# tomwhite/disq

Hardware: AMD Instinct MI355X
Metric: decompressed BAM GB/s + reads/sec (whole node) at 1/2/4/8 MI355X (higher is better)
Workload: dtype u8

## Files before the change

disq_amd/csrc/dq_inflate3.hip:

```cpp
#include "dq_inflate_core.h"
#include "dq_internal.h"

#include <mutex>
#include <vector>

namespace dq {
namespace {

using namespace dqi;

#define DQ_HD __device__ __host__ __attribute__((always_inline)) inline

#ifndef DQ_BLK_WG
#define DQ_BLK_WG 512
#endif
constexpr int WG = DQ_BLK_WG;
static_assert(WG % 128 == 0 && WG >= 512 && WG <= 1024, "whole waves on every SIMD");
constexpr int NWV = WG / 64;
constexpr int NDEC = WG;
constexpr uint32_t OV_DEFAULT = 96;
#ifndef DQ_TAIL_OV
#define DQ_TAIL_OV OV_DEFAULT
#endif
constexpr int OUTCAP = 65536 + 24;
#ifndef DQ_CSTEP
#define DQ_CSTEP 0
#endif
#ifndef DQ_RES_NB
#define DQ_RES_NB (WG == 512 ? 4 : 2)
#endif
#ifndef DQ_RES_G
#define DQ_RES_G 1
#endif
#ifndef DQ_RES_QUAD
#define DQ_RES_QUAD 1
#endif
constexpr int RES_NXT = DQ_RES_NB * DQ_RES_G * WG;
constexpr int NCARRY = (65536 + RES_NXT - 1) / RES_NXT + 1;


constexpr int LR = 10, DR = 8;
constexpr int LSB = 15 - LR, DSB = 15 - DR;
constexpr int LSLOTS = 16, DSLOTS = 4;
constexpr int MAXGRP = 64;
constexpr int T_LSUB = 1 << LR;
constexpr int T_DROOT = T_LSUB + LSLOTS * (1 << LSB);
constexpr int T_DSUB = T_DROOT + (1 << DR);
constexpr int T_END = T_DSUB + DSLOTS * (1 << DSB);
constexpr int HB_WORDS = 160;
constexpr uint16_t E_SLOW = 0x0080;
constexpr uint32_t LL_EOB = 0xF810, LL_BAD = 0xF910;
DQ_HD uint16_t ent_ll(uint32_t sym, uint32_t len) {
  if (sym < 256) return (uint16_t)(sym << 8 | len);
  if (sym == 256) return (uint16_t)(LL_EOB | len);
  if (sym > 285) return (uint16_t)(LL_BAD | len);
  const uint32_t k = sym - 257;
  const uint32_t x = (k < 8 || k == 28) ? 0u : (k - 4) >> 2;
  const uint32_t base = k < 8 ? k + 3 : k == 28 ? 258u : ((4u + (k & 3u)) << ((k - 4) >> 2)) + 3u;
  return (uint16_t)((base - 3) << 8 | x << 5 | 16u | len);
}
DQ_HD uint16_t ent_d(uint32_t d, uint32_t len) {
  if (d >= 30) return (uint16_t)(0x4000u | len);
  const uint32_t x = d < 4 ? 0u : (d - 2) >> 1;
  const uint32_t m = d < 2 ? d : 2u + (d & 1u), sh = d < 2 ? 0u : (d >> 1) - 1u;
  return (uint16_t)(m << 12 | sh << 8 | x << 4 | len);
}

enum : int32_t { F_EXIT = 0, F_EOB = 1, F_ERR = 2, F_END = 3 };

constexpr int TOUT = 4096;
constexpr int TAIL_MAX_BITS = 32768;
constexpr int TW = 4;
#ifndef DQ_ROOT_REG
#define DQ_ROOT_REG 1
#endif
#ifndef DQ_TAIL_HDR1
#define DQ_TAIL_HDR1 1
#endif
constexpr int T_NCK = 4;
#ifndef DQ_TAIL_SEG
#define DQ_TAIL_SEG 96
#endif
constexpr int TAIL_SEG_MIN = DQ_TAIL_SEG;
constexpr int TIM_W = 32;
struct TailDesc {
  int32_t pos;
  int32_t produced;
  uint32_t crc_raw;
  int32_t flag;
};

struct alignas(16) LdsI {
  static constexpr int kLSUB = T_LSUB, kDROOT = T_DROOT, kDSUB = T_DSUB;
  [[maybe_unused]] static constexpr int kTEND = T_END;
  static constexpr bool kPair = true;
  alignas(8) uint32_t bm[2048];
  union {
    struct {
      uint16_t T[T_END];
      HuffCanon hl, hd;
      uint16_t lend[16], dend[16];
      uint16_t lent[288];
      uint16_t dent[32];
      union {
        uint16_t pair[1 << LR];
        struct {
          uint8_t lens[320];
          uint8_t clen[20];
          uint16_t clt[128];
          union {
            struct {
              int32_t cntw[NWV];
              int32_t cnts[NWV];
              uint32_t ginfo[MAXGRP + 32];
              uint32_t cntp[8][8];
              uint16_t pref[320];
            };
            struct {
              uint8_t exitm[NWV][16];
              int32_t ent[NWV + 1];
              int32_t wt[NWV];
              int32_t lv[NWV];
              int32_t endp;
            };
          };
        } h;
      } x;
    } d;
    struct {
      uint16_t last_start[1024];
      uint16_t nxt[RES_NXT];
      int32_t carry_ms[NCARRY];
      uint32_t carry_desc[NCARRY];
    } r;
    uint32_t crc4[4][256];
  } u;
  int32_t misc[32];
  union {
    struct {
      int32_t wsum[16];
      int32_t small[8 * 7];
    };
    uint32_t scratch[16 + 8 * 7];
  };
  alignas(16) uint8_t out[OUTCAP];
};
static_assert(sizeof(((LdsI*)nullptr)->scratch) >= 64 * 4, "one emit dummy word per lane");
static_assert(offsetof(LdsI, out) < 65536 - 4096, "the tables' offsets fit the DS offset field");
static_assert(2 * sizeof(LdsI) <= 160 * 1024, "two workgroups per CU");
static_assert(HB_WORDS * 4 <= T_END * 2, "header staging fits the decode table");

__device__ inline uint32_t* emit_dummy(LdsI& L) { return L.scratch; }

__constant__ uint32_t c_crc4[4][256];
__constant__ uint32_t c_x2n[32];
__constant__ uint32_t c_x8n[TOUT + 1];
constexpr int CRC_SL = 4 * (((65536 / 4 + WG - 1) / WG) | 1);
static_assert(CRC_SL * WG >= 65536, "the slices cover the largest block");
__constant__ uint32_t c_slice_shift[WG];
__constant__ uint8_t c_clorder3[19] = {16, 17, 18, 0, 8, 7, 9, 6, 10, 5, 11, 4, 12, 3, 13, 2, 14, 1, 15};

enum { M_ERR = 0, M_SLOW = 1 , M_A = 4, M_LAST, M_MORE, M_MORE1,
       M_LQ0 = 15, M_LQN, M_DQ0, M_DQN, M_NEXT,
       M_LASTF, M_RCNT = 28 ,
       M_DIRTY = 30  };

template <class LT>
__device__ __attribute__((always_inline)) inline void set_err(LT& L, int32_t code) { atomicCAS(&L.misc[M_ERR], 0, code); }


#define DQ_AI __device__ __attribute__((always_inline)) inline

DQ_AI int tid_fresh() {
  int t = (int)threadIdx.x;
  asm volatile("" : "+v"(t));
  return t;
}

typedef uint32_t u32x4 __attribute__((ext_vector_type(4)));
DQ_AI void st_nt(uint4* d, uint4 v) {
  u32x4 x = {v.x, v.y, v.z, v.w};
  __builtin_nontemporal_store(x, reinterpret_cast<u32x4*>(d));
}

struct GSrc {
  const uint32_t* __restrict__ p;
#ifdef DQ_CHECKED
  uint32_t lim;
  uint32_t tag;
#endif
  DQ_AI uint32_t operator[](uint32_t i) const {
#ifdef DQ_CHECKED
    DQ_CHKV(i < lim, CHK_K2_BITS, tag | min(i - lim + 1, 4095u));
#endif
    return *reinterpret_cast<const uint32_t*>(reinterpret_cast<const uint8_t*>(p) + (i << 2));
  }
};

#ifndef DQ_BR64
#define DQ_BR64 0
#endif
#if DQ_BR64
struct BitR {
  uint64_t bb;
  uint32_t bc;
  uint32_t wp;
  uint32_t nw;
};
template <class S>
DQ_AI void br_init(BitR& r, const S& W, uint32_t bitpos) {
  const uint32_t wi = bitpos >> 5;
  const uint64_t lo = W[wi], hi = W[wi + 1];
  const uint32_t sh = bitpos & 31;
  r.bb = ((hi << 32) | lo) >> sh;
  r.bc = 64 - sh;
  r.wp = wi + 2;
  r.nw = W[r.wp];
}
template <class S>
DQ_AI void br_refill(BitR& r, const S& W) {
  const bool need = r.bc <= 32;
  r.bb |= (uint64_t)(need ? r.nw : 0u) << r.bc;
  r.bc += need ? 32u : 0u;
  r.wp += need ? 1u : 0u;
  r.nw = W[r.wp];
}
DQ_AI uint32_t br_pos(const BitR& r) { return r.wp * 32 - r.bc; }
DQ_AI uint32_t br_peek(const BitR& r) { return (uint32_t)r.bb; }
template <class S>
DQ_AI void br_take(BitR& r, const S&, uint32_t n) {
  r.bb >>= n;
  r.bc -= n;
}
#else
struct BitR {
  uint32_t p;
  uint32_t w0, w1;
  uint32_t nw;
};
template <class S>
DQ_AI void br_init(BitR& r, const S& W, uint32_t bitpos) {
  const uint32_t wi = bitpos >> 5;
  r.w0 = W[wi];
  r.w1 = W[wi + 1];
  r.nw = W[wi + 2];
  r.p = bitpos;
}
template <class S>
DQ_AI void br_refill(BitR&, const S&) {}
DQ_AI uint32_t br_pos(const BitR& r) { return r.p; }
DQ_AI uint32_t br_peek(const BitR& r) { return __builtin_amdgcn_alignbit(r.w1, r.w0, r.p); }
template <class S>
DQ_AI void br_take(BitR& r, const S& W, uint32_t n) {
  const uint32_t q = r.p + n;
  const bool c = (q ^ r.p) >= 32u;
  r.w0 = c ? r.w1 : r.w0;
  r.w1 = c ? r.nw : r.w1;
  r.p = q;
  r.nw = W[(q >> 5) + 2];
}
#endif
DQ_AI uint32_t peek_bits(const uint32_t* __restrict__ W, uint32_t pos, uint32_t n) {
  const uint32_t wi = pos >> 5;
  const uint64_t v = ((uint64_t)W[wi + 1] << 32) | W[wi];
  return (uint32_t)(v >> (pos & 31)) & ((1u << n) - 1);
}

template <class LT>
DQ_AI uint32_t load_desc(const LT& L, int a) {
  const uint32_t* w = reinterpret_cast<const uint32_t*>(L.out + (a & ~3));
  return __builtin_amdgcn_alignbyte(w[1], w[0], (uint32_t)a & 3u) & 0xffffffu;
}

DQ_AI uint32_t zx16(uint16_t v) {
#ifndef DQ_NO_ZX16
  uint32_t x = v;
  asm("" : "+v"(x));
  return x;
#else
  return v;
#endif
}

template <bool SLOW, class LT>
DQ_AI uint32_t ll_second(const LT& L, uint32_t e, uint32_t bb) {
  const uint32_t sb = (e >> 4) & 7;
  DQ_CHK(LT::kLSUB + (e >> 7) + ((bb >> LR) & ((1u << sb) - 1)) < (uint32_t)LT::kDROOT, CHK_K2_TABLE);
  if (!SLOW) return L.u.d.T[LT::kLSUB + (e >> 7) + ((bb >> LR) & ((1u << sb) - 1))];
  if (sb) return L.u.d.T[LT::kLSUB + (e >> 7) + ((bb >> LR) & ((1u << sb) - 1))];
  if (!(e & E_SLOW)) return 0u;
  int l = 0;
  const int k = canon_decode(bb, L.u.d.hl, LR + 1, &l);
  return k < 0 ? 0u : L.u.d.lent[k];
}
template <bool SLOW, class LT>
DQ_AI uint32_t d_second(const LT& L, uint32_t e, uint32_t bb) {
  const uint32_t sb = (e >> 4) & 7;
  DQ_CHK(LT::kDSUB + (e >> 7) + ((bb >> DR) & ((1u << sb) - 1)) < (uint32_t)LT::kTEND, CHK_K2_TABLE);
  if (!SLOW) return L.u.d.T[LT::kDSUB + (e >> 7) + ((bb >> DR) & ((1u << sb) - 1))];
  if (sb) return L.u.d.T[LT::kDSUB + (e >> 7) + ((bb >> DR) & ((1u << sb) - 1))];
  if (!(e & E_SLOW)) return 0u;
  int l = 0;
  const int k = canon_decode(bb, L.u.d.hd, DR + 1, &l);
  return k < 0 ? 0u : L.u.d.dent[k];
}


template <bool SLOW, class S, class LT>
DQ_AI bool dsym(BitR& r, const S& W, const LT& L, uint32_t p, uint32_t lim,
                uint32_t& len, uint32_t& dist, uint32_t& lit2, bool& is_m, uint32_t& e) {
  br_refill(r, W);
  uint32_t bb = br_peek(r);
  const uint32_t ri = bb & ((1u << LR) - 1);
  e = L.u.d.T[ri];
  uint32_t pe = 0;
  if constexpr (LT::kPair) pe = zx16(L.u.d.x.pair[ri]);
  if ((e & 15) == 0) e = ll_second<SLOW>(L, e, bb);
  const uint32_t nb = e & 15;
  const uint32_t lx = __builtin_amdgcn_ubfe(e, 5, 3);
  is_m = (e & 16) != 0;
  len = (e >> 8) + (is_m ? 3u : 0u) + __builtin_amdgcn_ubfe(bb, nb, lx);
  const bool two = pe != 0 && p + nb < lim;
  lit2 = two ? pe >> 8 : 0xffffffffu;
  br_take(r, W, nb + lx + (two ? (pe & 15) : 0u));
  br_refill(r, W);
  bb = br_peek(r);
  uint32_t e2 = zx16(L.u.d.T[LT::kDROOT + (bb & ((1u << DR) - 1))]);
  if (is_m && (e2 & 15) == 0) e2 = d_second<SLOW>(L, e2, bb);
  const uint32_t nb2 = e2 & 15, dx = __builtin_amdgcn_ubfe(e2, 4, 4);
  dist = (__builtin_amdgcn_ubfe(e2, 12, 2) << __builtin_amdgcn_ubfe(e2, 8, 4)) + 1u +
         __builtin_amdgcn_ubfe(bb, nb2, dx);
  br_take(r, W, is_m ? nb2 + dx : 0u);
  return (SLOW && nb == 0) || (e & 0xFEF0u) == 0xF810u ||
         (is_m && ((SLOW && nb2 == 0) || (e2 & 0x4000u)));
}
DQ_AI uint32_t stop_end(uint32_t e, uint32_t p) {
  return (e & 15) != 0 && (e & 0xFFF0u) == LL_EOB ? p + (e & 15) : 0xffffffffu;
}

enum : int32_t { F_DEAD = 4 };

constexpr int NCK_DEFAULT = 8;
constexpr uint32_t CKI_DEFAULT = 48;

template <bool SLOW, class S, class LT>
DQ_AI int run_seg(const S& W, const LT& L, uint32_t start, uint32_t sB,
                  uint32_t sE, uint32_t endbits, int32_t* Bp, int32_t* Ep, int32_t* cntp,
                  uint32_t* ck, int ckstride, uint32_t CKI, int NCK) {
  BitR r;
  br_init(r, W, start);
  uint32_t p = br_pos(r);
  uint32_t len = 0, dist = 0, lit2, e = 0;
  bool m;
  const uint32_t sBe = min(sB, endbits);
  while (p < sBe) {
    if (dsym<SLOW>(r, W, L, p, sBe, len, dist, lit2, m, e)) {
      len = stop_end(e, p);
      *Ep = (int32_t)(len != 0xffffffffu ? len : p);
      *Bp = -1;
      *cntp = 0;
      return F_DEAD;
    }
    p = br_pos(r);
  }
  if (p < sB) {
    *Ep = (int32_t)p;
    *Bp = -1;
    *cntp = 0;
    return F_DEAD;
  }
  const int32_t B = (int32_t)p;
  int32_t cnt = 0;
  int f;
  uint32_t thr = ck ? sB + CKI : 0xffffffffu;
  uint32_t* const dummy = const_cast<uint32_t*>(L.scratch) + (tid_fresh() & 15);
  uint32_t* ckp = ck;
  const uint32_t* const cke = ck + NCK * ckstride;
  const uint32_t sEe = min(sE, endbits);
  bool stopped;
  for (;;) {
    const bool cross = p >= thr;
    const bool st = cross && ckp < cke;
    *(st ? ckp : dummy) = ((p - sB) << 16) | (uint32_t)cnt;
    ckp += st ? ckstride : 0;
    thr += cross ? CKI : 0u;
    stopped = false;
    if (p >= sEe) break;
    stopped = true;
    if (dsym<SLOW>(r, W, L, p, min(thr, sEe), len, dist, lit2, m, e)) break;
    cnt += m ? (int32_t)len : (lit2 != 0xffffffffu ? 2 : 1);
    p = br_pos(r);
  }
  if (stopped) {
    len = stop_end(e, p);
    *Ep = (int32_t)(len != 0xffffffffu ? len : p);
    f = len != 0xffffffffu ? F_EOB : F_ERR;
  } else {
    *Ep = (int32_t)p;
    f = p >= sE ? F_EXIT : F_END;
  }
  *Bp = B;
  *cntp = cnt;
  return f;
}

template <bool SLOW, class S, class LT>
DQ_AI int run_redo(const S& W, const LT& L, uint32_t s0, uint32_t sB,
                   uint32_t sE, uint32_t endbits, const uint32_t* ck, int ckstride, int32_t se,
                   int32_t sc, int32_t* Ep, int32_t* cntp, uint32_t CKI, int NCK, int* jm = nullptr) {
  BitR r;
  br_init(r, W, s0);
  int32_t cnt = 0;
  int f;
  uint32_t thr = ck ? sB + CKI : 0xffffffffu;
  uint32_t cur = ck ? ck[0] : 0xffffffffu;
  const uint32_t* ckq = ck;
  const uint32_t* const ckl = ck + (NCK - 1) * ckstride;
  const uint32_t sEe = min(sE, endbits);
  int j = 0;
  int why;
  uint32_t p, len = 0, e = 0;
  for (;;) {
    p = br_pos(r);
    const bool cross = p >= thr;
    const bool merge = cross && (cur >> 16) == p - sB;
    why = merge ? 1 : 0;
    if (p >= sEe || merge) break;
    const bool more = ckq < ckl;
    if (jm) j += cross ? 1 : 0;
    ckq += cross && more ? ckstride : 0;
    const uint32_t nxt = ck ? *ckq : 0xffffffffu;
    thr += cross ? CKI : 0u;
    cur = cross ? (more ? nxt : 0xffffffffu) : cur;
    uint32_t dist = 0, lit2;
    bool m;
    why = 2;
    if (dsym<SLOW>(r, W, L, p, min(thr, sEe), len, dist, lit2, m, e)) break;
    cnt += m ? (int32_t)len : (lit2 != 0xffffffffu ? 2 : 1);
  }
  if (why == 1) {
    *Ep = se >> 3;
    f = se & 7;
    cnt += sc - (int32_t)(cur & 0xffffu);
    if (jm) *jm = j;
  } else if (why == 2) {
    len = stop_end(e, p);
    *Ep = (int32_t)(len != 0xffffffffu ? len : p);
    f = len != 0xffffffffu ? F_EOB : F_ERR;
  } else {
    *Ep = (int32_t)p;
    f = p >= sE ? F_EXIT : F_END;
  }
  *cntp = cnt;
  return f;
}

template <bool SLOW, class S, class LT>
DQ_AI void emit_seg(const S& W, LT& L, uint32_t start, uint32_t target,
                    uint32_t endbits, int32_t p, int32_t isize, int sh, int32_t ibase = 0) {
  typedef volatile __attribute__((address_space(3))) uint8_t lds8;
  uint32_t* const dummy32 = emit_dummy(L) + (tid_fresh() & 63);
  lds8* const dummy1 = (lds8*)dummy32 - 1;
  lds8* const dummy2 = (lds8*)dummy32 - 2;
  BitR r;
  br_init(r, W, start);
  const uint32_t te = min(target, endbits);
  int32_t obase = sh - ibase;
  asm("" : "+v"(obase));
  bool bad = false;
  for (;;) {
    const uint32_t q = br_pos(r);
    if (q >= te || p >= isize) break;
    uint32_t len = 0, dist = 0, lit2;
    bool m;
    uint32_t e;
    const bool stop = dsym<SLOW>(r, W, L, q, te, len, dist, lit2, m, e);
    const bool far = m && (int32_t)dist > p;
    bad = far && !stop;
    if (stop || far) break;
    const bool two = !m && lit2 != 0xffffffffu && p + 1 < isize;
    DQ_CHK(p >= ibase && sh + p - ibase + 2 < (int)sizeof(L.out) &&
               ((p - ibase) >> 5) < (int)(sizeof(L.bm) / 4), CHK_K2_IMAGE);
    const uint32_t desc = (dist - 1) | ((len - 3) << 15);
    lds8* const o = (lds8*)(L.out + (obase + p));
    o[0] = (uint8_t)(m ? desc : len);
    (m || two ? o : dummy1)[1] = (uint8_t)(m ? desc >> 8 : lit2);
    (m ? o : dummy2)[2] = (uint8_t)(desc >> 16);
    atomicOr(m ? &L.bm[(p - ibase) >> 5] : dummy32, 1u << ((p - ibase) & 31));
    p += m ? (int32_t)len : (two ? 2 : 1);
  }
  if (bad) set_err(L, ST_BAD_DIST);
}

__device__ inline uint32_t gf2_mulmod(uint32_t a, uint32_t b) {
  uint32_t p = 0;
#pragma unroll
  for (int i = 31; i >= 0; i--) {
    p ^= ((a >> i) & 1u) ? b : 0u;
    b = (b >> 1) ^ ((b & 1u) ? 0xEDB88320u : 0u);
  }
  return p;
}

DQ_AI int wave_incl_scan(int v, int) {
  v += __builtin_amdgcn_update_dpp(0, v, 0x111, 0xf, 0xf, false);
  v += __builtin_amdgcn_update_dpp(0, v, 0x112, 0xf, 0xf, false);
  v += __builtin_amdgcn_update_dpp(0, v, 0x114, 0xf, 0xf, false);
  v += __builtin_amdgcn_update_dpp(0, v, 0x118, 0xf, 0xf, false);
  v += __builtin_amdgcn_update_dpp(0, v, 0x142, 0xa, 0xf, false);
  v += __builtin_amdgcn_update_dpp(0, v, 0x143, 0xc, 0xf, false);
  return v;
}
DQ_AI int wave_incl_or(int v) {
  v |= __builtin_amdgcn_update_dpp(0, v, 0x111, 0xf, 0xf, false);
  v |= __builtin_amdgcn_update_dpp(0, v, 0x112, 0xf, 0xf, false);
  v |= __builtin_amdgcn_update_dpp(0, v, 0x114, 0xf, 0xf, false);
  v |= __builtin_amdgcn_update_dpp(0, v, 0x118, 0xf, 0xf, false);
  v |= __builtin_amdgcn_update_dpp(0, v, 0x142, 0xa, 0xf, false);
  v |= __builtin_amdgcn_update_dpp(0, v, 0x143, 0xc, 0xf, false);
  return v;
}
DQ_AI uint32_t wave_incl_xor(uint32_t v) {
  v ^= (uint32_t)__builtin_amdgcn_update_dpp(0, (int)v, 0x111, 0xf, 0xf, false);
  v ^= (uint32_t)__builtin_amdgcn_update_dpp(0, (int)v, 0x112, 0xf, 0xf, false);
  v ^= (uint32_t)__builtin_amdgcn_update_dpp(0, (int)v, 0x114, 0xf, 0xf, false);
  v ^= (uint32_t)__builtin_amdgcn_update_dpp(0, (int)v, 0x118, 0xf, 0xf, false);
  v ^= (uint32_t)__builtin_amdgcn_update_dpp(0, (int)v, 0x142, 0xa, 0xf, false);
  v ^= (uint32_t)__builtin_amdgcn_update_dpp(0, (int)v, 0x143, 0xc, 0xf, false);
  return v;
}
DQ_AI int wave_incl_max(int v) {
  v = max(v, __builtin_amdgcn_update_dpp(-1, v, 0x111, 0xf, 0xf, false));
  v = max(v, __builtin_amdgcn_update_dpp(-1, v, 0x112, 0xf, 0xf, false));
  v = max(v, __builtin_amdgcn_update_dpp(-1, v, 0x114, 0xf, 0xf, false));
  v = max(v, __builtin_amdgcn_update_dpp(-1, v, 0x118, 0xf, 0xf, false));
  v = max(v, __builtin_amdgcn_update_dpp(-1, v, 0x142, 0xa, 0xf, false));
  v = max(v, __builtin_amdgcn_update_dpp(-1, v, 0x143, 0xc, 0xf, false));
  return v;
}
DQ_AI uint64_t lanes_below(int lane) { return lane ? (~0ull >> (64 - lane)) : 0ull; }

template <int W0, int NW, int R>
DQ_AI int canon_from_counts(LdsI& L, HuffCanon& h, uint16_t* end, int32_t* q0p, int32_t* qnp) {
  const int l = tid_fresh() & 63;
  const bool in = l >= 1 && l <= 15;
  uint32_t pk = 0;
#pragma unroll
  for (int w = W0; w < W0 + NW; w++) pk += in ? L.u.d.x.h.cntp[w][l >> 1] : 0u;
  const int c = in ? (int)((pk >> (16 * (l & 1))) & 0xffffu) : 0;
  const int offi = wave_incl_scan(c, l);
  const int tt = in ? c << (16 - l) : 0;
  const int code = in ? (int)((uint32_t)(wave_incl_scan(tt, l) - tt) >> (16 - l)) : 0;
  const int left = in ? (1 << l) - (code + c) : 0;
  const uint64_t over = __ballot(in && left < 0);
  const uint64_t used = __ballot(c > 0);
  const int maxl = used ? 63 - __clzll(used) : 0;
  const int left15 = __builtin_amdgcn_readlane(left, 15);
  if (l < 16) {
    h.first[l] = (uint16_t)code;
    h.count[l] = (uint16_t)c;
    h.offs[l] = (uint16_t)(offi - c);
    if (in && l <= R) end[l] = (uint16_t)((code + c) << (R - l));
  }
  if (l == 0) {
    *q0p = __builtin_amdgcn_readlane(offi, R);
    *qnp = __builtin_amdgcn_readlane(offi, 15);
  }
  if (over) return ST_BAD_TABLE;
  if (maxl > 0 && left15 > 0 && maxl != 1) return ST_BAD_TABLE;
  return 0;
}

template <int R, class LT>
DQ_AI uint16_t root_entry(const LT& L, const HuffCanon& h, const uint16_t* end,
                          const uint16_t* ent, uint32_t r) {
  int l = 1;
#pragma unroll
  for (int k = 1; k <= R; k++) l += (uint32_t)end[k] <= r ? 1 : 0;
  if (l > R) return 0;
  const int q = (int)h.offs[l] + (int)(r >> (R - l)) - (int)h.first[l];
  return ent[q];
}
template <int R>
struct RootEnds {
  uint32_t e[R + 1];
// ... 499 lines not shown
      const int f = slow ? run_seg<true>(gsrc, L, start, sB, sE, endbits, &B, &E, &c,
                                         CK ? CK + t : nullptr, nl, CKI, NCK)
                         : run_seg<false>(gsrc, L, start, sB, sE, endbits, &B, &E, &c,
                                          CK ? CK + t : nullptr, nl, CKI, NCK);
      AB[t] = B;
      AE[t] = (E << 3) | f;
      AC[t] = c;
      SE[t] = (E << 3) | f;
      SC[t] = c;
    }
    __syncthreads();
    TST(2);
#ifdef DQ_CHECKED
    gsrc.tag = 2u << 12;
#endif
    for (int round = 0; round <= nl; round++) {
      bool need = false;
      int32_t st = 0;
      if (t > 0 && t < nl) {
        const int32_t pe = AE[t - 1];
        st = pe >> 3;
        need = (pe & 7) == F_EXIT && AB[t] != st;
      }
      int32_t* rc = &L.misc[M_RCNT + (round & 1)];
      if (need) {
        const int r = atomicAdd(rc, 1);
        DQ_CHK(r < nl, CHK_K2_LANES);
        LS[r] = t;
        ST[r] = st;
      }
      if (t == 0) {
        L.misc[M_RCNT + ((round + 1) & 1)] = 0;
        L.misc[M_DIRTY + (round & 1)] = 0;
      }
      __syncthreads();
      const int nneed = *rc;
      if (nneed == 0) break;
      TCOUNT(10);
      const bool hi = __builtin_amdgcn_readfirstlane(t) < __builtin_amdgcn_readfirstlane(nneed);
      if (hi) __builtin_amdgcn_s_setprio(3);
      if (t < nneed) {
        const int lt = LS[t];
        const uint32_t s0 = (uint32_t)ST[t];
        const uint32_t sE = lt == nl - 1 ? 0xffffffffu : a + (uint32_t)(lt + 1) * seg;
        int32_t E = 0, c = 0;
        int jmerge = -1;
        const uint32_t sB = a + (uint32_t)lt * seg;
        const int f = slow ? run_redo<true>(gsrc, L, s0, sB, sE, endbits, CK ? CK + lt : nullptr,
                                            nl, SE[lt], SC[lt], &E, &c, CKI, NCK,
                                            TIMING ? &jmerge : nullptr)
                           : run_redo<false>(gsrc, L, s0, sB, sE, endbits, CK ? CK + lt : nullptr,
                                             nl, SE[lt], SC[lt], &E, &c, CKI, NCK,
                                             TIMING ? &jmerge : nullptr);
        const int32_t ae = (E << 3) | f;
        if (ae != AE[lt]) L.misc[M_DIRTY + (round & 1)] = 1;
        AB[lt] = (int32_t)s0;
        AE[lt] = ae;
        AC[lt] = c;
        if (TIMING) {
          atomicAdd(&L.misc[21], 1);
          if (jmerge >= 0) {
            atomicAdd(&L.misc[23], 1);
            atomicAdd(&L.misc[24], jmerge);
          } else {
            const int sf = SE[lt] & 7;
            atomicAdd(&L.misc[sf == F_ERR || sf == F_EOB ? 25 : sf == F_EXIT ? 26 : 27], 1);
          }
        }
      }
      if (hi) __builtin_amdgcn_s_setprio(0);
      __syncthreads();
      if (L.misc[M_DIRTY + (round & 1)] == 0) break;
    }
    TST(3);

    int32_t myB = 0, myE = 0, myF = F_DEAD, myC = 0;
    if (t < nl) {
      myB = AB[t];
      myE = AE[t] >> 3;
      myF = AE[t] & 7;
      myC = AC[t];
    }
    if (t < nl && myF != F_EXIT) atomicMin(&L.misc[M_LAST], t);
    __syncthreads();
    const int last = L.misc[M_LAST];
    const int32_t cv = t <= last ? myC : 0;
    const int32_t incl = wave_incl_scan(cv, lane);
    if (lane == 63) L.wsum[wv] = incl;
    if (t == last) {
      L.misc[M_NEXT] = myE;
      L.misc[M_LASTF] = myF;
    }
    __syncthreads();
    int32_t woff = 0;
    for (int w = 0; w < wv; w++) woff += L.wsum[w];
    const int32_t myoff = produced + woff + incl - cv;
    int32_t total = 0;
    for (int w = 0; w < WG / 64; w++) total += L.wsum[w];
    const bool full = produced + total >= isize;
    const int32_t fl = L.misc[M_LASTF];
    if (!full && fl != F_EOB && t == 0) L.misc[M_ERR] = fl == F_ERR ? ST_BAD_CODE : ST_SHORT;
    __syncthreads();
    TST(4);
    if (L.misc[M_ERR]) break;
#ifdef DQ_CHECKED
    gsrc.tag = 3u << 12;
#endif
    if (t <= last && myoff < isize) {
      const uint32_t sE = t == nl - 1 ? 0xffffffffu : a + (uint32_t)(t + 1) * seg;
      if (slow) emit_seg<true>(gsrc, L, (uint32_t)myB, sE, endbits, myoff, isize, sh);
      else emit_seg<false>(gsrc, L, (uint32_t)myB, sE, endbits, myoff, isize, sh);
    }
    const int32_t nextpos = L.misc[M_NEXT];
    __syncthreads();
    TST(5);
    produced = min(isize, produced + total);
    if (TIMING && t == 0) {
      if (tacc[22] == 0)
        for (int i = 0; i < 6; i++) tacc[16 + i] = tacc[i];
      tacc[22] += 1;
    }
    if (full || bfinal) break;
    pos = (uint32_t)nextpos;
    if (tails && isize - produced <= TOUT && endbits - pos <= (uint32_t)TAIL_MAX_BITS) {
      deferred = true;
      break;
    }
  }
  __syncthreads();
  int32_t err = L.misc[M_ERR];
  if (!err && !deferred && produced != isize) err = ST_SHORT;
  const int32_t rsize = deferred ? produced : isize;
  if (deferred && t == 0) {
    TailDesc td;
    td.pos = (int32_t)pos;
    td.produced = produced;
    td.crc_raw = 0;
    td.flag = 1;
    tails[blockIdx.x] = td;
  }
  if (err) {
    if (t == 0) status[b] = err;
    return;
  }
  const uint64_t* bm64 = reinterpret_cast<const uint64_t*>(L.bm);
  {
    int ls[2];
    int run = -1;
#pragma unroll
    for (int k = 0; k < 2; k++) {
      const uint64_t m = 2 * t + k < 1024 ? bm64[min(2 * t + k, 1023)] : 0ull;
      if (m) run = 64 * (2 * t + k) + 63 - __clzll(m);
      ls[k] = run;
    }
    const int wm = wave_incl_max(run);
    if (lane == 63) L.wsum[wv] = wm;
    int ex = __shfl_up(wm, 1, 64);
    if (lane == 0) ex = -1;
    __syncthreads();
    for (int w = 0; w < wv; w++) ex = max(ex, L.wsum[w]);
#pragma unroll
    for (int k = 0; k < 2; k++) {
      const int v = max(ex, ls[k]);
      if (WG == 512 || 2 * t + k < 1024) L.u.r.last_start[2 * t + k] = v < 0 ? (uint16_t)0xffff : (uint16_t)v;
    }
    __syncthreads();
  }
  uint8_t* dstU = U + ub;
  const uint8_t* O = L.out + sh;
  const int head = min((16 - sh) & 15, rsize);
  int32_t lines_done = 0;
  constexpr int CH = G * WG;
  constexpr int BATCH = NB * CH;
  constexpr int NE = NB * G;
  constexpr bool CSTEP = (DQ_CSTEP != 0 && G > 1) || CH % 512 != 0;
  static_assert(BATCH <= RES_NXT, "the batch's next-pointers fit the resolve scratch");
  static_assert((65536 + BATCH - 1) / BATCH <= NCARRY, "one carry slot per batch");
  static_assert(CSTEP || CH / 512 <= G, "the G ordered steps of a chunk cover it");
  constexpr bool QUAD = G == 4 && DQ_RES_QUAD != 0;
  constexpr bool HYB = G == 1 && NB == 4 && WG == 512 && !CSTEP && DQ_RES_QUAD != 0;
  constexpr int GK = HYB ? 1 : NB, GCH = HYB ? BATCH : CH;
  static_assert(!(QUAD || HYB) || offsetof(LdsI, u.r.nxt) % 8 == 0, "a group's next pointers are one 64-bit word");
  constexpr bool INR = 65536 % BATCH == 0;
  uint16_t* nxt = L.u.r.nxt;
  auto pack16 = [](int32_t lo, int32_t hi) {
    return __builtin_amdgcn_perm((uint32_t)hi, (uint32_t)lo, 0x05040100u);
  };
  auto med3 = [](int32_t a, int32_t b, int32_t c) { return max(min(a, b), min(max(a, b), c)); };
  auto store_nxt4 = [&](int off, uint32_t lo, uint32_t hi) {
    const uint2 v = make_uint2(lo, hi);
    __builtin_memcpy(__builtin_assume_aligned(nxt + off, 8), &v, 8);
  };
  auto first_hop = [&](int32_t b0, int32_t cms, uint32_t cdesc, int32_t* fr, int32_t* xs,
                       bool& pending) {
    pending = false;
    if constexpr (QUAD || HYB) {
#pragma unroll
      for (int k = 0; k < GK; k++) {
        const int32_t g0 = b0 + k * GCH + 4 * t;
        const int w = INR ? g0 >> 6 : min(g0 >> 6, 1023);
        DQ_CHK(w >= 0 && w < 1024, CHK_K2_LAST);
        const uint64_t m = bm64[w];
        const int32_t ls = w ? (int32_t)zx16(L.u.r.last_start[w - 1]) : 0xffff;
        const uint32_t bit = (uint32_t)g0 & 60u;
        const uint64_t below = m & ~(~0ull << bit);
        const int32_t prev = below ? (g0 | 63) - (int32_t)__clzll(below) : ls;
        const uint32_t nib = (uint32_t)(m >> bit) & 15u;
        DQ_CHK(g0 >= rsize || ((0x0317u >> nib) & 1u), CHK_K2_BM);
        const bool hasB = nib != 0;
        const int32_t A = (nib & 1u) ? g0 : prev;
        const int32_t Bs = hasB ? g0 + 31 - (int32_t)__clz(nib) : A;
        const uint32_t ldA = load_desc(L, sh + (INR ? A : min(A, 65535)));
        const uint32_t ldB = load_desc(L, sh + (INR ? Bs : min(Bs, 65535)));
        const uint32_t dA = A < b0 ? cdesc : ldA;
        const uint32_t dB = hasB ? ldB : dA;
        const int32_t D1A = (int32_t)(dA & 0x7fff), D1B = (int32_t)(dB & 0x7fff);
        const int32_t remA = A == 0xffff ? 0 : rsize - A;
        const int32_t limA = med3(remA, 0, (int32_t)(dA >> 15) + 3);
        const int32_t limB = med3(hasB ? rsize - Bs : remA, 0, (int32_t)(dB >> 15) + 3);
        const int32_t sbk = b0 + k * GCH + (CSTEP ? 0 : ((4 * t) & ~511));
        int32_t f4[4];
#pragma unroll
        for (int i = 0; i < 4; i++) {
          const int32_t x = g0 + i;
          const bool useB = i == 0 ? false : i == 3 ? true : x >= Bs;
          const int32_t ms = useB ? Bs : A, lim = useB ? limB : limA, D1 = useB ? D1B : D1A;
          const int32_t jj = x - ms;
          const bool copy = (uint32_t)jj < (uint32_t)lim;
          int32_t src = (int32_t)((uint32_t)D1 ^ ~0u) + x;
          if (__builtin_expect(__any(copy && jj > D1), 0)) {
            const int32_t D = D1 + 1;
            const int32_t q = (int32_t)((float)jj * __builtin_amdgcn_rcpf((float)D));
            int32_t r = jj - q * D;
            r = r >= D ? r - D : r;
            src = ms - D + r;
          }
          DQ_CHK(!copy || (src >= 0 && src < x), CHK_K2_SRC);
          f4[i] = copy ? src : x;
          if constexpr (QUAD) {
            const bool done = !copy || src < sbk;
            fr[4 * k + i] = f4[i];
            xs[4 * k + i] = done ? x : src;
            pending = pending || !done;
          }
        }
        DQ_CHK(k * GCH + 4 * t + 3 < BATCH, CHK_K2_NXT);
        store_nxt4(k * GCH + 4 * t, pack16(f4[0], f4[1]), pack16(f4[2], f4[3]));
      }
      return;
    }
    uint64_t mw[NB];
    int32_t lsv[NB];
#pragma unroll
    for (int k = 0; k < NB; k++) {
      const int32_t g0 = b0 + k * CH + G * t;
      const int w = min(g0 >> 6, 1023);
      DQ_CHK(w >= 0 && w - 1 < 1024, CHK_K2_LAST);
      mw[k] = bm64[w];
      lsv[k] = w ? (int32_t)zx16(L.u.r.last_start[w - 1]) : 0xffff;
    }
    int32_t msv[NE];
    uint32_t da[NB], db[NB];
#pragma unroll
    for (int k = 0; k < NB; k++) {
      const int32_t g0 = b0 + k * CH + G * t;
#pragma unroll
      for (int i = 0; i < G; i++) {
        const uint64_t mi = mw[k] & (~0ull >> (63 - ((g0 + i) & 63)));
        msv[k * G + i] = mi ? (g0 | 63) - (int32_t)__clzll(mi) : lsv[k];
      }
      da[k] = load_desc(L, sh + min(msv[k * G], 65535));
      db[k] = G > 1 ? load_desc(L, sh + min(msv[k * G + G - 1], 65535)) : da[k];
    }
#pragma unroll
    for (int k = 0; k < NB; k++) {
      const int32_t g0 = b0 + k * CH + G * t;
      const int32_t sbk = b0 + k * CH + (CSTEP ? 0 : ((G * t) & ~511));
#pragma unroll
      for (int i = 0; i < G; i++) {
        const int e = k * G + i;
        const int32_t x = g0 + i, ms = msv[e];
        const bool before = ms < b0;
        const uint32_t desc = before ? cdesc : (ms == msv[k * G + G - 1] ? db[k] : da[k]);
        const int32_t len = (int32_t)(desc >> 15) + 3, D1 = (int32_t)(desc & 0x7fff);
        const bool copy = x < rsize && ms != 0xffff && (!before || ms == cms) && x < ms + len;
        const int32_t jj = x - ms;
        int32_t src = (int32_t)((uint32_t)D1 ^ ~0u) + x;
        if (__builtin_expect(__any(copy && jj > D1), 0)) {
          const int32_t D = D1 + 1;
          const int32_t q = (int32_t)((float)jj * __builtin_amdgcn_rcpf((float)D));
          int32_t r = jj - q * D;
          r = r >= D ? r - D : r;
          src = ms - D + r;
        }
        DQ_CHK(!copy || (src >= 0 && src < x), CHK_K2_SRC);
        const bool done = !copy || src < sbk;
        fr[e] = copy ? src : x;
        xs[e] = done ? x : src;
        pending = pending || !done;
        nxt[x - b0] = (uint16_t)(copy ? src : x);
      }
    }
  };
  auto adopt = [&](int32_t b0, int32_t* fr, int32_t* xs, bool& pending) {
    int32_t qv[NE];
#pragma unroll
    for (int e = 0; e < NE; e++) qv[e] = (int32_t)zx16(nxt[(e / G) * CH + G * t + e % G]);
    pending = false;
#pragma unroll
    for (int e = 0; e < NE; e++) {
      const int32_t x = b0 + (e / G) * CH + G * t + e % G;
      const int32_t sbk = b0 + (e / G) * CH + ((G * t) & ~511);
      const int32_t q = qv[e];
      const bool done = q == x || q < sbk;
      fr[e] = q;
      xs[e] = done ? x : q;
      pending = pending || !done;
    }
  };
  auto jump_round = [&](int32_t b0, int32_t* fr, int32_t* xs, bool& pending) {
    int32_t qv[NE];
#pragma unroll
    for (int e = 0; e < NE; e++) {
      DQ_CHK(xs[e] - b0 >= 0 && xs[e] - b0 < BATCH, CHK_K2_NXT);
      qv[e] = (int32_t)zx16(nxt[xs[e] - b0]);
    }
    bool any = false;
#pragma unroll
    for (int e = 0; e < NE; e++) {
      const int32_t own = (e / G) * CH + G * t + e % G;
      const int32_t p = xs[e], q = qv[e];
      const bool pd = p != b0 + own;
      const int32_t sbk = b0 + (e / G) * CH + (CSTEP ? 0 : ((G * t) & ~511));
      const bool fin = pd && (q == p || q < sbk);
      const bool go = pd && !fin;
      fr[e] = fin ? q : fr[e];
      xs[e] = go ? q : b0 + own;
      any = any || go;
      if constexpr (!QUAD) nxt[own] = (uint16_t)q;
    }
    if constexpr (QUAD) {
#pragma unroll
      for (int k = 0; k < NB; k++)
        store_nxt4(k * CH + 4 * t, pack16(qv[4 * k], qv[4 * k + 1]), pack16(qv[4 * k + 2], qv[4 * k + 3]));
    }
    pending = any;
  };
  int32_t frA[NE], xsA[NE];
  bool pendA = false;
  int32_t cms = -1;
  uint32_t cdesc = 0;
  first_hop(0, cms, cdesc, frA, xsA, pendA);
  if (t < (rsize + BATCH - 1) / BATCH) {
    int32_t ncms = -1;
    uint32_t ncdesc = 0;
    const int32_t x = (t + 1) * BATCH - 1;
    if (x + 1 < rsize) {
      const uint64_t m = bm64[x >> 6];
      const int32_t ms = m ? (x | 63) - (int32_t)__clzll(m) : (int32_t)L.u.r.last_start[(x >> 6) - 1];
      if (ms != 0xffff) {
        const uint32_t desc = load_desc(L, sh + ms);
        if (ms + (int32_t)(desc >> 15) + 3 > x + 1) {
          ncms = ms;
          ncdesc = desc;
        }
      }
    }
    L.u.r.carry_ms[t] = ncms;
    L.u.r.carry_desc[t] = ncdesc;
  }
  __syncthreads();
  if constexpr (HYB) adopt(0, frA, xsA, pendA);
  for (int hop = 0; pendA && hop < WG + 2; hop++) jump_round(0, frA, xsA, pendA);
  for (int32_t bs = 0; bs < rsize; bs += BATCH) {
    const uint64_t tb0 = TIMING ? __builtin_amdgcn_s_memtime() : 0;
    const int32_t nbs = bs + BATCH;
    const bool more = nbs < rsize;
    __syncthreads();
    const int32_t ncms = more ? L.u.r.carry_ms[bs / BATCH] : -1;
    const uint32_t ncdesc = more ? L.u.r.carry_desc[bs / BATCH] : 0u;
    int32_t frB[NE], xsB[NE];
    bool pendB = false;
    if (more) first_hop(nbs, ncms, ncdesc, frB, xsB, pendB);
    const uint64_t tb1 = TIMING ? __builtin_amdgcn_s_memtime() : 0;
#pragma unroll
    for (int k = 0; k < NB; k++) {
#pragma unroll
      for (int j = 0; j < (CSTEP ? 1 : G); j++) {
        const bool mine = CSTEP || ((G * t) >> 9) == j;
        const int32_t g0 = bs + k * CH + G * t;
        uint8_t v[G];
        if (mine)
#pragma unroll
          for (int i = 0; i < G; i++) {
            DQ_CHK(g0 + i >= rsize || (frA[k * G + i] >= 0 && frA[k * G + i] <= g0 + i), CHK_K2_SRC);
            v[i] = O[INR ? frA[k * G + i] : min(frA[k * G + i], 65535)];
          }
        if constexpr (HYB)
          if (k == 1 && more) adopt(nbs, frB, xsB, pendB);
        if ((k > 0 || j > 0) && pendB) jump_round(nbs, frB, xsB, pendB);
        if constexpr (QUAD && INR) {
          if (mine) {
            const uint32_t lo = (uint32_t)v[0] | (uint32_t)v[1] << 8;
            const uint32_t hi = (uint32_t)v[2] | (uint32_t)v[3] << 8;
            uint8_t* const p = L.out + sh + g0;
            if ((sh & 3) == 0) {
              const uint32_t w4 = lo | hi << 16;
              __builtin_memcpy(__builtin_assume_aligned(p, 4), &w4, 4);
            } else if ((sh & 3) == 2) {
              const uint16_t a2 = (uint16_t)lo, b2 = (uint16_t)hi;
              __builtin_memcpy(__builtin_assume_aligned(p, 2), &a2, 2);
              __builtin_memcpy(__builtin_assume_aligned(p + 2, 2), &b2, 2);
            } else {
              const uint16_t m2 = (uint16_t)(v[1] | v[2] << 8);
              p[0] = v[0];
              __builtin_memcpy(__builtin_assume_aligned(p + 1, 2), &m2, 2);
              p[3] = v[3];
            }
          }
        } else {
          if (mine)
#pragma unroll
            for (int i = 0; i < G; i++)
              if (g0 + i < rsize) L.out[sh + g0 + i] = v[i];
        }
        __syncthreads();
      }
    }
    if (pendB) jump_round(nbs, frB, xsB, pendB);
    const uint64_t tb2 = TIMING ? __builtin_amdgcn_s_memtime() : 0;
    const int32_t c1 = min(rsize, nbs);
    const int32_t lines_to = c1 >= head ? (c1 - head) / 16 : 0;
    if (!(sflags & 1)) {
      for (int32_t k = lines_done + t; k < lines_to; k += WG) {
        const uint4 v = *reinterpret_cast<const uint4*>(O + head + 16 * k);
        uint4* d = reinterpret_cast<uint4*>(dstU + head + 16 * k);
        if (sflags & 2) st_nt(d, v);
        else *d = v;
      }
      lines_done = lines_to;
    }
    const uint64_t tb3 = TIMING ? __builtin_amdgcn_s_memtime() : 0;
    for (int hop = 0; pendB && hop < WG + 2; hop++) jump_round(nbs, frB, xsB, pendB);
#pragma unroll
    for (int e = 0; e < NE; e++) frA[e] = frB[e];
    cms = ncms;
    cdesc = ncdesc;
    if (TIMING && t == 0) {
      tacc[9] += tb1 - tb0;
      tacc[12] += tb2 - tb1;
      tacc[13] += tb3 - tb2;
      tacc[14] += __builtin_amdgcn_s_memtime() - tb3;
      tacc[15] += 1;
    }
  }
  if (sflags & 1) {
    const int32_t lines_to = rsize >= head ? (rsize - head) / 16 : 0;
    for (int32_t k = t; k < lines_to; k += WG) {
      const uint4 v = *reinterpret_cast<const uint4*>(O + head + 16 * k);
      uint4* d = reinterpret_cast<uint4*>(dstU + head + 16 * k);
      if (sflags & 2) st_nt(d, v);
      else *d = v;
    }
    lines_done = lines_to;
  }
  uint32_t ct0 = 0, ct1 = 0, cshift = 0, cinit = 0, cwant = 0;
  if (verify_crc) {
    ct0 = (&c_crc4[0][0])[t];
    ct1 = t + WG < 1024 ? (&c_crc4[0][0])[t + WG] : 0u;
    cshift = c_slice_shift[WG - 1 - t];
    if (t == 0) {
      cinit = crc_init[rsize];
      const uint8_t* tr = C + cpos + csize - 8;
      cwant = (uint32_t)tr[0] | ((uint32_t)tr[1] << 8) | ((uint32_t)tr[2] << 16) | ((uint32_t)tr[3] << 24);
    }
  }
  static_assert(2 * WG >= 1024, "at most two CRC table words per thread");
  for (int x = t; x < head; x += WG) dstU[x] = O[x];
  for (int x = head + 16 * lines_done + t; x < rsize; x += WG) dstU[x] = O[x];
  TST(6);
  if (verify_crc) {
    __syncthreads();
    if (t < 1024) (&L.u.crc4[0][0])[t] = ct0;
    if (t + WG < 1024) (&L.u.crc4[0][0])[t + WG] = ct1;
    __syncthreads();
    const int32_t e = rsize - (WG - 1 - t) * CRC_SL;
    const int32_t s0 = max(0, e - CRC_SL);
    uint32_t cr = 0;
    if (e > 0) {
      int32_t x = s0;
      while (x < e && ((sh + x) & 3)) cr = L.u.crc4[0][(cr ^ O[x++]) & 0xff] ^ (cr >> 8);
      for (; x + 4 <= e; x += 4) {
        const uint32_t v = cr ^ *reinterpret_cast<const uint32_t*>(O + x);
        cr = L.u.crc4[3][v & 0xff] ^ L.u.crc4[2][(v >> 8) & 0xff] ^ L.u.crc4[1][(v >> 16) & 0xff] ^
             L.u.crc4[0][v >> 24];
      }
      while (x < e) cr = L.u.crc4[0][(cr ^ O[x++]) & 0xff] ^ (cr >> 8);
      cr = gf2_mulmod(cshift, cr);
    }
    cr = wave_incl_xor(cr);
    if (lane == 63) L.wsum[wv] = (int32_t)cr;
    __syncthreads();
    if (t == 0) {
      uint32_t x = 0;
      for (int w = 0; w < WG / 64; w++) x ^= (uint32_t)L.wsum[w];
      if (deferred) {
        tails[blockIdx.x].crc_raw = x;
      } else {
        const uint32_t crc = (x ^ cinit) ^ 0xffffffffu;
        if (crc != cwant) status[b] = ST_CRC;
      }
    }
  }
  TST(7);
  if (TIMING && t == 0)
    for (int i = 0; i < 24; i++) tim[(int64_t)blockIdx.x * TIM_W + i] = tacc[i];
  if (TIMING && t == 0)
    for (int i = 0; i < 7; i++) tim[(int64_t)blockIdx.x * TIM_W + 24 + i] = (uint64_t)L.misc[21 + i];
}

struct alignas(16) LdsW {
  static constexpr int kLSUB = 0, kDROOT = 1 << LR, kDSUB = 0, kTEND = (1 << LR) + (1 << DR);
  static constexpr bool kPair = false;
  union {
    struct {
      uint16_t T[kTEND];
      HuffCanon hl, hd;
      uint16_t lend[16], dend[16];
      uint16_t lent[288];
      uint16_t dent[32];
      union {
        struct {
          uint8_t lens[320];
          uint8_t clen[20];
          uint16_t clt[128];
          int32_t cnt[32];
          int32_t run[32];
        } h;
      } x;
    } d;
    uint32_t crc4[4][256];
  } u;
  alignas(16) uint8_t out[TOUT + 32];
  alignas(8) uint32_t bm[TOUT / 32];
  uint32_t ck[T_NCK * 64];
  int32_t misc[8];
  uint32_t scratch[16];
};
static_assert(HB_WORDS * 4 <= LdsW::kTEND * 2, "header staging fits the decode table");
static_assert(4 * 4 * sizeof(LdsW) <= 160 * 1024, "four tails per workgroup, four workgroups per CU");
DQ_AI uint32_t* emit_dummy(LdsW& L) { return L.ck; }

DQ_AI uint32_t read_lengths_wave(LdsW& L, uint32_t P, int nlen, int ndist, uint32_t endbits,
                                 uint32_t hbase) {
  const uint32_t* hb = reinterpret_cast<const uint32_t*>(L.u.d.T);
  auto& H = L.u.d.x.h;
  const int lane = tid_fresh() & 63;
  const int total = nlen + ndist;
  int have = 0, prev = -1, entry = 0;
  for (uint32_t W0 = P;; W0 += 64) {
    if (W0 > endbits) {
      set_err(L, ST_OVERREAD);
      return W0;
    }
    const uint32_t p = W0 + (uint32_t)lane;
    const uint32_t wi = min((p >> 5) - hbase, (uint32_t)HB_WORDS - 2);
    const uint32_t v = (uint32_t)((((uint64_t)hb[wi + 1] << 32) | hb[wi]) >> (p & 31));
    const uint32_t ent = H.clt[v & 127];
    const uint32_t cl = ent & 7, sy = ent >> 3;
    const uint32_t ex = sy == 16 ? 2u : sy == 17 ? 3u : sy == 18 ? 7u : 0u;
    const int xv = (int)((v >> cl) & ((1u << ex) - 1));
    const int rep = sy < 16 ? 1 : sy == 16 ? 3 + xv : sy == 17 ? 3 + xv : 11 + xv;
    const int adv = cl ? (int)(cl + ex) : 0;
    int J[6];
    J[0] = adv ? min(lane + adv, 64) : lane;
#pragma unroll
    for (int k = 1; k < 6; k++) {
      const int y = __shfl(J[k - 1], J[k - 1] & 63, 64);
      J[k] = J[k - 1] >= 64 ? 64 : y;
    }
    int pk = entry;
#pragma unroll
    for (int k = 0; k < 6; k++) {
      const int y = __shfl(J[k], pk & 63, 64);
      if ((lane >> k) & 1) pk = pk >= 64 ? 64 : y;
    }
    const bool onp = pk < 64;
    const int src = pk & 63;
    const int s_rep = __shfl(rep, src, 64), s_adv = __shfl(adv, src, 64);
    const int s_sy = __shfl((int)sy, src, 64);
    const int pprev = __shfl_up(pk, 1, 64);
    const bool real = onp && (lane == 0 || pprev != pk);
    const bool bad = real && s_adv == 0;
    const int r = real && !bad ? s_rep : 0;
    const int incl = wave_incl_scan(r, lane);
    const int key = wave_incl_max(real && !bad && s_sy != 16 ? ((lane + 1) << 5) | (s_sy < 16 ? s_sy : 0) : 0);
    const int kprev = __shfl_up(key, 1, 64);
    const int before = lane == 0 ? 0 : kprev;
    const int val = s_sy < 16 ? s_sy : s_sy == 16 ? (before > 0 ? (before & 31) : prev) : 0;
    const bool take = real && have + incl - r < total;
    if (__any((take && bad) || (take && s_sy == 16 && val < 0) || (take && have + incl > total))) {
      set_err(L, ST_BAD_TABLE);
      return W0;
    }
    if (take && val != 0)
      for (int i = have + incl - r; i < have + incl; i++) H.lens[i < nlen ? i : 288 + i - nlen] = (uint8_t)val;
    const uint64_t tk = __ballot(take);
    const int lastk = tk ? 63 - (int)__clzll(tk) : -1;
    if (lastk >= 0 && __shfl(have + incl, lastk, 64) >= total) {
      __builtin_amdgcn_wave_barrier();
      return W0 + (uint32_t)__shfl(pk + s_adv, lastk, 64);
    }
    const uint64_t rm = __ballot(real);
    const int lastr = rm ? 63 - (int)__clzll(rm) : -1;
    if (lastr < 0 || __shfl((int)bad, lastr, 64)) {
      set_err(L, ST_BAD_TABLE);
      return W0;
    }
    have = __shfl(have + incl, lastr, 64);
    const int kl = __shfl(key, 63, 64);
    prev = kl > 0 ? (kl & 31) : prev;
    entry = __shfl(pk + s_adv, lastr, 64) - 64;
  }
}

DQ_AI void build_tables_wave(LdsW& L, int nlen, int ndist) {
  const int lane = tid_fresh() & 63;
  auto& H = L.u.d.x.h;
  if (lane < 32) {
    H.cnt[lane] = 0;
    H.run[lane] = 0;
  }
  __builtin_amdgcn_wave_barrier();
  for (int k = lane; k < 320; k += 64) {
    const bool isl = k < 288;
    const int len = isl ? (k < nlen ? H.lens[k] : 0) : (k - 288 < ndist ? H.lens[k] : 0);
    if (len) atomicAdd(&H.cnt[(isl ? 0 : 16) + len], 1);
  }
  __builtin_amdgcn_wave_barrier();
  __builtin_amdgcn_fence(__ATOMIC_SEQ_CST, "wavefront");
  int e = 0;
  {
    const int l = lane & 15;
    const bool in = lane < 32 && l >= 1;
    const int c = in ? H.cnt[lane] : 0;
    int offi = wave_incl_scan(c, lane);
    const int tt = in ? c << (16 - l) : 0;
    int cs = wave_incl_scan(tt, lane);
    const int base_o = __shfl(offi, 15, 64), base_c = __shfl(cs, 15, 64);
    if (lane >= 16) {
      offi -= base_o;
      cs -= base_c;
    }
    const int code = in ? (int)((uint32_t)(cs - tt) >> (16 - l)) : 0;
    const int left = in ? (1 << l) - (code + c) : 0;
    const bool isd = lane >= 16;
    HuffCanon& h = isd ? L.u.d.hd : L.u.d.hl;
    uint16_t* end = isd ? L.u.d.dend : L.u.d.lend;
    const int R = isd ? DR : LR;
    if (lane < 32) {
      h.first[l] = (uint16_t)code;
      h.count[l] = (uint16_t)c;
      h.offs[l] = (uint16_t)(offi - c);
      if (in && l <= R) end[l] = (uint16_t)((code + c) << (R - l));
    }
    const uint64_t over = __ballot(in && left < 0);
    const uint64_t used = __ballot(c > 0);
    const int left15l = __shfl(left, 15, 64), left15d = __shfl(left, 31, 64);
    const uint64_t ul = used & 0xffffull, ud = (used >> 16) & 0xffffull;
    const int maxll = ul ? 63 - __clzll(ul) : 0, maxld = ud ? 63 - __clzll(ud) : 0;
    if (over) e = ST_BAD_TABLE;
    if (maxll > 0 && left15l > 0 && maxll != 1) e = ST_BAD_TABLE;
    if (maxld > 0 && left15d > 0 && maxld != 1) e = ST_BAD_TABLE;
    const int ql0 = __shfl(offi, LR, 64), qln = __shfl(offi, 15, 64);
    const int qd0 = __shfl(offi, 16 + DR, 64), qdn = __shfl(offi, 31, 64);
    if (lane == 0) L.misc[M_SLOW] = (qln > ql0 || qdn > qd0) ? 1 : 0;
  }
  if (e) {
    if (lane == 0) set_err(L, e);
    return;
  }
  __builtin_amdgcn_wave_barrier();
  const uint64_t below = lanes_below(lane);
  for (int k0 = 0; k0 < 320; k0 += 64) {
    const int k = k0 + lane;
    const bool isl = k < 288;
    const int sym = isl ? k : k - 288;
    const int len = k < 320 ? (isl ? (k < nlen ? H.lens[k] : 0) : (sym < ndist ? H.lens[k] : 0)) : 0;
    const int key = (isl ? 0 : 16) + len;
    uint64_t peers = ~0ull;
#pragma unroll
    for (int bt = 0; bt < 5; bt++) {
      const uint64_t bl = __ballot((key >> bt) & 1);
      peers &= ((key >> bt) & 1) ? bl : ~bl;
    }
    const int run0 = H.run[key];
    const int rank = run0 + __popcll(peers & below);
    __builtin_amdgcn_wave_barrier();
    if (len && (peers >> lane) == 1ull) H.run[key] = run0 + __popcll(peers);
    if (len) {
      const HuffCanon& hh = isl ? L.u.d.hl : L.u.d.hd;
      const int q = hh.offs[len] + rank;
      if (isl) L.u.d.lent[q] = ent_ll((uint32_t)sym, (uint32_t)len);
      else L.u.d.dent[q] = ent_d((uint32_t)sym, (uint32_t)len);
    }
    __builtin_amdgcn_wave_barrier();
  }
  __builtin_amdgcn_wave_barrier();
  const bool lslow = L.u.d.hl.count[11] + L.u.d.hl.count[12] + L.u.d.hl.count[13] +
                         L.u.d.hl.count[14] + L.u.d.hl.count[15] > 0;
  const bool dslow = L.u.d.hd.count[9] + L.u.d.hd.count[10] + L.u.d.hd.count[11] + L.u.d.hd.count[12] +
                         L.u.d.hd.count[13] + L.u.d.hd.count[14] + L.u.d.hd.count[15] > 0;
#if DQ_ROOT_REG
  const RootEnds<LR> le = root_ends<LR>(L.u.d.lend);
  const RootEnds<DR> de = root_ends<DR>(L.u.d.dend);
#endif
  for (int i = lane; i < (1 << LR); i += 64) {
#if DQ_ROOT_REG
    const uint16_t v = root_entry_r<LR>(L.u.d.hl, le, L.u.d.lent, bitrev((uint32_t)i, LR));
#else
    const uint16_t v = root_entry<LR>(L, L.u.d.hl, L.u.d.lend, L.u.d.lent, bitrev((uint32_t)i, LR));
#endif
    L.u.d.T[i] = v ? v : lslow ? E_SLOW : (uint16_t)(LL_BAD | 1u);
  }
  for (int i = lane; i < (1 << DR); i += 64) {
#if DQ_ROOT_REG
    const uint16_t v = root_entry_r<DR>(L.u.d.hd, de, L.u.d.dent, bitrev((uint32_t)i, DR));
#else
    const uint16_t v = root_entry<DR>(L, L.u.d.hd, L.u.d.dend, L.u.d.dent, bitrev((uint32_t)i, DR));
#endif
    L.u.d.T[LdsW::kDROOT + i] = v ? v : dslow ? E_SLOW : (uint16_t)0x4001u;
  }
  __builtin_amdgcn_wave_barrier();
}

DQ_AI uint32_t x8n_tail(uint32_t n) {
  uint32_t p = 1u << 31;
  for (int k = 3; n; n >>= 1, k++)
    if (n & 1) p = gf2_mulmod(c_x2n[k & 31], p);
  return p;
}

template <bool TIMING>
__global__ __launch_bounds__(64 * TW, 4) void inflate_tail_kernel(
    const uint8_t* __restrict__ C, const int64_t* __restrict__ blk_pos,
    const int32_t* __restrict__ blk_csize, const int32_t* __restrict__ blk_usize,
// ... 535 lines not shown
```

Before: 184.5.

## Track pointer-jump state as byte offsets with wave-uniform liveness in resolver

In the hybrid back-reference resolver, per-element state is now kept as precomputed LDS byte offsets relative to each slice, with a single unsigned compare deciding pending status. Pending status is tracked as a wave-uniform ballot mask instead of a per-lane bool, and the batch loop bound is made scalar via readfirstlane. An optional slice mode skips jump rounds for slices with no pending lanes. The aim is fewer VALU address computations and divergent branches per jump round, at the cost of extra ballots and more complex control flow.

```diff
diff --git a/disq_amd/csrc/dq_inflate3.hip b/disq_amd/csrc/dq_inflate3.hip
--- a/disq_amd/csrc/dq_inflate3.hip
+++ b/disq_amd/csrc/dq_inflate3.hip
@@ -34,6 +34,9 @@
 #endif
 #ifndef DQ_RES_QUAD
 #define DQ_RES_QUAD 1
+#endif
+#ifndef DQ_RES_SLICE
+#define DQ_RES_SLICE 0
 #endif
 constexpr int RES_NXT = DQ_RES_NB * DQ_RES_G * WG;
 constexpr int NCARRY = (65536 + RES_NXT - 1) / RES_NXT + 1;
@@ -281,6 +284,12 @@
   return v;
 #endif
 }
+DQ_AI uint32_t zx32(uint32_t x) {
+#ifndef DQ_NO_ZX16
+  asm("" : "+v"(x));
+#endif
+  return x;
+}
 
 template <bool SLOW, class LT>
 DQ_AI uint32_t ll_second(const LT& L, uint32_t e, uint32_t bb) {
@@ -1386,22 +1395,6 @@
       }
     }
   };
-  auto adopt = [&](int32_t b0, int32_t* fr, int32_t* xs, bool& pending) {
-    int32_t qv[NE];
-#pragma unroll
-    for (int e = 0; e < NE; e++) qv[e] = (int32_t)zx16(nxt[(e / G) * CH + G * t + e % G]);
-    pending = false;
-#pragma unroll
-    for (int e = 0; e < NE; e++) {
-      const int32_t x = b0 + (e / G) * CH + G * t + e % G;
-      const int32_t sbk = b0 + (e / G) * CH + ((G * t) & ~511);
-      const int32_t q = qv[e];
-      const bool done = q == x || q < sbk;
-      fr[e] = q;
-      xs[e] = done ? x : q;
-      pending = pending || !done;
-    }
-  };
   auto jump_round = [&](int32_t b0, int32_t* fr, int32_t* xs, bool& pending) {
     int32_t qv[NE];
 #pragma unroll
@@ -1430,8 +1423,63 @@
     }
     pending = any;
   };
+  constexpr bool SLICE = DQ_RES_SLICE != 0;
+  const uint32_t own2 = 2u * (uint32_t)t;
+  auto LB = [](int e) { return 2u << e; };
+  auto nxt_at = [&](int e, uint32_t ra) {
+    return reinterpret_cast<uint16_t*>(reinterpret_cast<char*>(nxt) + e * (CH * 2) + ra);
+  };
+  auto adopt_live = [&](int32_t b0, int32_t* fr, uint32_t* ra, uint32_t& live) {
+    int32_t qv[NE];
+#pragma unroll
+    for (int e = 0; e < NE; e++) qv[e] = (int32_t)zx16(*nxt_at(e, own2));
+    const uint32_t cb = 2u * (uint32_t)-b0;
+    live = 0;
+    uint64_t anym = 0;
+#pragma unroll
+    for (int e = 0; e < NE; e++) {
+      const uint32_t na = ((uint32_t)qv[e] << 1) + (cb - 2u * e * CH);
+      const bool pend = na < own2;
+      fr[e] = qv[e];
+      ra[e] = pend ? na : own2;
+      if constexpr (SLICE) live |= __ballot(pend) != 0 ? LB(e) : 0u;
+      else anym |= __ballot(pend);
+    }
+    if constexpr (!SLICE) live = anym != 0 ? LB(0) : 0u;
+  };
+  auto jump_round_live = [&](int32_t b0, int32_t* fr, uint32_t* ra, uint32_t& live) {
+    const uint32_t cb = 2u * (uint32_t)-b0;
+#pragma unroll
+    for (int e = 0; e < NE; e++)
+      if (!SLICE || (live & LB(e))) {
+        DQ_CHK(ra[e] < 2u * CH && !(ra[e] & 1u), CHK_K2_NXT);
+        fr[e] = *nxt_at(e, ra[e]);
+      }
+    uint32_t nl = 0;
+    uint64_t anym = 0;
+#pragma unroll
+    for (int e = 0; e < NE; e++)
+      if (!SLICE || (live & LB(e))) {
+        const uint32_t q = zx32(fr[e]);
+        fr[e] = (int32_t)q;
+        const uint32_t na = (q << 1) + (cb - 2u * e * CH);
+        const bool pd = ra[e] != own2, lt = na < ra[e];
+        ra[e] = pd && lt ? na : own2;
+        if constexpr (SLICE) nl |= (__ballot(pd) & __ballot(lt)) != 0 ? LB(e) : 0u;
+        else anym |= __ballot(pd) & __ballot(lt);
+        *nxt_at(e, own2) = (uint16_t)q;
+      }
+    live = SLICE ? nl : anym != 0 ? LB(0) : 0u;
+  };
   int32_t frA[NE], xsA[NE];
+  uint32_t raA[NE];
   bool pendA = false;
+  uint32_t liveA = 0;
+  auto left = [&](bool pending, uint32_t live) { return HYB ? live != 0 : pending; };
+  auto round = [&](int32_t b0, int32_t* fr, int32_t* xs, uint32_t* ra, bool& pending, uint32_t& live) {
+    if constexpr (HYB) jump_round_live(b0, fr, ra, live);
+    else jump_round(b0, fr, xs, pending);
+  };
   int32_t cms = -1;
   uint32_t cdesc = 0;
   first_hop(0, cms, cdesc, frA, xsA, pendA);
@@ -1454,17 +1502,20 @@
     L.u.r.carry_desc[t] = ncdesc;
   }
   __syncthreads();
-  if constexpr (HYB) adopt(0, frA, xsA, pendA);
-  for (int hop = 0; pendA && hop < WG + 2; hop++) jump_round(0, frA, xsA, pendA);
-  for (int32_t bs = 0; bs < rsize; bs += BATCH) {
+  if constexpr (HYB) adopt_live(0, frA, raA, liveA);
+  for (int hop = 0; left(pendA, liveA) && hop < WG + 2; hop++) round(0, frA, xsA, raA, pendA, liveA);
+  const int32_t rsize_u = HYB ? __builtin_amdgcn_readfirstlane(rsize) : rsize;
+  for (int32_t bs = 0; bs < rsize_u; bs += BATCH) {
     const uint64_t tb0 = TIMING ? __builtin_amdgcn_s_memtime() : 0;
     const int32_t nbs = bs + BATCH;
-    const bool more = nbs < rsize;
+    const bool more = nbs < rsize_u;
     __syncthreads();
     const int32_t ncms = more ? L.u.r.carry_ms[bs / BATCH] : -1;
     const uint32_t ncdesc = more ? L.u.r.carry_desc[bs / BATCH] : 0u;
     int32_t frB[NE], xsB[NE];
+    uint32_t raB[NE];
     bool pendB = false;
+    uint32_t liveB = 0;
     if (more) first_hop(nbs, ncms, ncdesc, frB, xsB, pendB);
     const uint64_t tb1 = TIMING ? __builtin_amdgcn_s_memtime() : 0;
 #pragma unroll
@@ -1481,8 +1532,8 @@
             v[i] = O[INR ? frA[k * G + i] : min(frA[k * G + i], 65535)];
           }
         if constexpr (HYB)
-          if (k == 1 && more) adopt(nbs, frB, xsB, pendB);
-        if ((k > 0 || j > 0) && pendB) jump_round(nbs, frB, xsB, pendB);
+          if (k == 1 && more) adopt_live(nbs, frB, raB, liveB);
+        if ((k > 0 || j > 0) && left(pendB, liveB)) round(nbs, frB, xsB, raB, pendB, liveB);
         if constexpr (QUAD && INR) {
           if (mine) {
             const uint32_t lo = (uint32_t)v[0] | (uint32_t)v[1] << 8;
@@ -1511,7 +1562,7 @@
         __syncthreads();
       }
     }
-    if (pendB) jump_round(nbs, frB, xsB, pendB);
+    if (left(pendB, liveB)) round(nbs, frB, xsB, raB, pendB, liveB);
     const uint64_t tb2 = TIMING ? __builtin_amdgcn_s_memtime() : 0;
     const int32_t c1 = min(rsize, nbs);
     const int32_t lines_to = c1 >= head ? (c1 - head) / 16 : 0;
@@ -1525,7 +1576,7 @@
       lines_done = lines_to;
     }
     const uint64_t tb3 = TIMING ? __builtin_amdgcn_s_memtime() : 0;
-    for (int hop = 0; pendB && hop < WG + 2; hop++) jump_round(nbs, frB, xsB, pendB);
+    for (int hop = 0; left(pendB, liveB) && hop < WG + 2; hop++) round(nbs, frB, xsB, raB, pendB, liveB);
 #pragma unroll
     for (int e = 0; e < NE; e++) frA[e] = frB[e];
     cms = ncms;
```

Result: faster. 191.7, median of 6 (+3.9%).
